# 3DAnimals/3DAnimals

Measured on AMD Instinct MI355X. Metric: train images/sec fwd+bwd @256x256 b16, higher is better.
Workload: dtype f32

## Files before the change

### 3danimals_amd/_lib.py

```python
from __future__ import annotations

import ctypes
import os

import torch

_HERE = os.path.dirname(os.path.abspath(__file__))
LIB_PATH = os.environ.get("A3D_LIB") or os.path.join(_HERE, "lib", "liba3d_hip.so")

_c_int, _c_float, _c_size_t, _p = ctypes.c_int, ctypes.c_float, ctypes.c_size_t, ctypes.c_void_p

SIGNATURES = {
    "a3d_version": (_c_int, []),
    "a3d_last_error": (ctypes.c_char_p, []),
    "a3d_bw_probe_fill": (_c_int, [_p, ctypes.c_int64, _p]),
    "a3d_bw_probe_read": (_c_int, [_p, ctypes.c_int64, _p, _p]),
    "a3d_dmtet_scratch_bytes": (_c_size_t, [_c_int, _c_int]),
    "a3d_dmtet_count": (_c_int, [_p, _p, _p, _c_int, _c_int, _p, _p, _p, _c_int, _c_int, _p, _p, _c_int, _p, _c_int, _p]),
    "a3d_dmtet_count_ordered": (_c_int, [_p, _c_int, _c_int, _c_int, _p, _p, _p, _p, _c_int, _p, _c_int, _p]),
    "a3d_dmtet_word_group_slots": (_c_int, []),
    "a3d_dmtet_word_group_bits": (_c_int, []),
    "a3d_dmtet_block_items": (_c_int, []),
    "a3d_dmtet_vertex_scratch_bytes": (_c_size_t, [_c_int]),
    "a3d_dmtet_gather_rows": (_c_int, [_p, _p, ctypes.c_int64, ctypes.c_int64, _c_int, _p, _p]),
# ... 125 lines not shown


class EstimateBonesArgs(ctypes.Structure):

    _fields_ = [("size", ctypes.c_uint32), ("N", ctypes.c_int32), ("pos", _p), ("bones", _p), ("nearest", _p), ("ok", _p), ("V", ctypes.c_int32),
                ("n_body", ctypes.c_int32), ("n_leg", ctypes.c_int32), ("body_mode_y_plus", ctypes.c_int32), ("use_y_threshold", ctypes.c_int32),
                ("y_threshold", ctypes.c_float), ("attach", ctypes.c_int32 * 4), ("blend", ctypes.c_float * 17), ("ramp", ctypes.c_float * 9), ("workspace", _p)]


class GbAux(ctypes.Structure):

    _fields_ = [("size", ctypes.c_uint32), ("reserved", ctypes.c_int32), ("tex_out", _p), ("img_out", _p), ("rows", ctypes.c_int64),
                ("pad_to", ctypes.c_int64)]


class DmtetEmitOpts(ctypes.Structure):

    _fields_ = [("size", ctypes.c_uint32), ("Nv", ctypes.c_int32), ("vertex_scratch", _p), ("surf_idx", _p), ("g_sdf_to_clear", _p), ("tri32", _p),
                ("topo_count", _p), ("topo_adj", _p), ("device_counts", _p), ("n_surf", ctypes.c_int32), ("topo_stride", ctypes.c_int32),
                ("use_block_lists", ctypes.c_int32), ("n_edge_blocks_listed", ctypes.c_int32), ("n_tet_blocks_listed", ctypes.c_int32),
                ("surf_bucket", ctypes.c_int32), ("surf_pts", _p)]


class TexDesc(ctypes.Structure):

    _fields_ = [("size", ctypes.c_uint32), ("C", ctypes.c_int32), ("tex_batch", ctypes.c_int32), ("filter", ctypes.c_int32), ("boundary", ctypes.c_int32),
                ("levels", ctypes.c_int32), ("height", ctypes.c_int32 * 16), ("width", ctypes.c_int32 * 16), ("level", _p * 16), ("grad", _p * 16)]


class EnvDesc(ctypes.Structure):

    _fields_ = [("size", ctypes.c_uint32), ("N", ctypes.c_int32), ("roughness", ctypes.c_float), ("costheta_cutoff", ctypes.c_float), ("src", _p),
                ("dst", _p), ("bounds", _p), ("area", _p)]


class BsdfDesc(ctypes.Structure):

    _fields_ = [("size", ctypes.c_uint32), ("op", ctypes.c_int32), ("variant", ctypes.c_int32), ("min_roughness", ctypes.c_float),
                ("ndim", ctypes.c_int32), ("reserved", ctypes.c_int32), ("shape", ctypes.c_int64 * 4), ("seg", ctypes.c_int64), ("in", _p * 6),
                ("stride", ctypes.c_int64 * 24), ("cstride", ctypes.c_int64 * 6), ("out", _p), ("scratch", _p), ("g_out", _p),
                ("g_mode", ctypes.c_int32 * 6), ("seg_div", ctypes.c_int64 * 6), ("g_in", _p * 6), ("g_final", _p * 6)]


BSDF_SIGNATURES = {
    "a3d_bsdf_rows": (ctypes.c_int64, [_p]),
    "a3d_bsdf_fwd": (_c_int, [_p, _p]),
    "a3d_bsdf_bwd": (_c_int, [_p, _p]),
    "a3d_image_loss_fwd": (_c_int, [_p, _p]),
    "a3d_image_loss_bwd": (_c_int, [_p, _p]),
}
BSDF_TILE = 1024
BSDF_MAX_DIMS = 4

ABI_VERSION = 404
_lib = None


class A3DError(RuntimeError):
    pass


def lib():
    global _lib
    if _lib is None:
        if not os.path.exists(LIB_PATH):
            raise A3DError(
                f"{LIB_PATH} is missing: build it with `python 3danimals_amd/csrc/build.py` "
                "(or __graft_entry__.build()).  There is no CPU fallback for the HIP hot path."
            )
        handle = ctypes.CDLL(LIB_PATH)
        for name, (res, args) in list(SIGNATURES.items()) + list(BSDF_SIGNATURES.items()):
            fn = getattr(handle, name)
            fn.restype, fn.argtypes = res, args
        if handle.a3d_version() != ABI_VERSION:
            raise A3DError(f"{LIB_PATH} has ABI version {handle.a3d_version()}, this package binds version {ABI_VERSION}: rebuild it "
                           "with `python 3danimals_amd/csrc/build.py`")
        _lib = handle
    return _lib


class KernelTimer:

    active = None

    def __init__(self):
        self.records = {}

    def __enter__(self):
        KernelTimer.active = self
        return self

    def __exit__(self, *exc):
        KernelTimer.active = None
        return False

    def summary(self):
        torch.cuda.synchronize()
        out = {}
        for name, pairs in self.records.items():
            ms = [a.elapsed_time(b) for a, b in pairs]
            out[name] = (len(ms), sum(ms) / max(len(ms), 1))
        return out


GUARD = int(os.environ.get("A3D_GUARD", "0") or 0)
GUARD_BYTES = 256
_GUARD_BYTE = 0xA5
_guard_live = []
guard_stats = dict(checks=0, buffers_checked=0, allocations=0)


def set_guard(level):
    global GUARD
    import importlib

    prev, GUARD = GUARD, int(level)
    ops = importlib.import_module(__package__ + ".ops")
    ops.torch = GuardedTorch(torch) if GUARD else torch
    if not GUARD:
        _guard_live.clear()
    return prev


def guarded_empty(shape, dtype, device, zero=False, site=""):
# ... 238 lines not shown
```

### 3danimals_amd/csrc/build.py

```python
import os
import subprocess
import sys
from concurrent.futures import ThreadPoolExecutor

HERE = os.path.dirname(os.path.abspath(__file__))
PKG = os.path.dirname(HERE)
LIB_DIR = os.path.join(PKG, "lib")
LIB = os.path.join(LIB_DIR, "liba3d_hip.so")
OBJ_DIR = os.path.join(HERE, "build")

SOURCES = {
    "common.hip": [],
    "dmtet.hip": ["-ffp-contract=off"],
    "skin.hip": [],
    "bones.hip": [],
    "normals.hip": ["-ffp-contract=off"],
    "raster.hip": ["-ffp-contract=off"],
    "cover.hip": [],
    "shade.hip": ["-ffp-contract=off"],
    "interp.hip": [],
    "gbuffer.hip": [],
    "segsum.hip": [],
    "losses.hip": [],
    "embed.hip": ["-ffp-contract=off"],
    "gemm.hip": [],
    "antialias.hip": ["-ffp-contract=off"],
    "topology.hip": [],
    "xfm.hip": ["-ffp-contract=off"],
    "texture.hip": ["-ffp-contract=off"],
    "envlight.hip": ["-ffp-contract=off"],
    "bsdf.hip": ["-ffp-contract=off"],
}
COMMON = ["--offload-arch=gfx950", "-O3", "-std=c++17", "-fPIC", "-fhip-fp32-correctly-rounded-divide-sqrt", "-Wall",
          "-Wno-unused-function"]


def _hipcc():
    for c in (os.environ.get("HIPCC"), "/opt/rocm/bin/hipcc", "hipcc"):
        if c and (os.path.isabs(c) and os.path.exists(c) or not os.path.isabs(c)):
            return c
    raise RuntimeError("hipcc not found")


def _stale(target, deps):
    if not os.path.exists(target):
        return True
    t = os.path.getmtime(target)
    return any(os.path.getmtime(d) > t for d in deps)


def build(force=False, verbose=True, profile=False, exp=False):
    assert not (profile and exp)
    lib = os.path.join(LIB_DIR, "liba3d_hip_prof.so") if profile else (os.path.join(LIB_DIR, "liba3d_hip_exp.so") if exp else LIB)
    obj_dir = os.path.join(OBJ_DIR, "prof") if profile else (os.path.join(OBJ_DIR, "exp") if exp else OBJ_DIR)
    os.makedirs(LIB_DIR, exist_ok=True)
    os.makedirs(obj_dir, exist_ok=True)
    hipcc = _hipcc()
    headers = sorted(os.path.join(HERE, f) for f in os.listdir(HERE) if f.endswith(".h")) + [os.path.join(os.path.dirname(PKG), "include", h) for h in ("a3d.h", "a3d_bsdf.h")] + [os.path.abspath(__file__)]
    jobs = []
    objs = []
    for src, extra in SOURCES.items():
        s = os.path.join(HERE, src)
        o = os.path.join(obj_dir, src.replace(".hip", ".o"))
        objs.append(o)
        if force or _stale(o, [s] + headers):
            jobs.append([hipcc, "-x", "hip", "-c", s, "-o", o] + COMMON + extra + (["-DA3D_PROFILE"] if profile else []) + (["-DA3D_EXPERIMENT"] if exp else []))

    def run(cmd):
        if verbose:
            print(" ".join(cmd), flush=True)
        subprocess.check_call(cmd)

    with ThreadPoolExecutor(max_workers=min(8, max(1, len(jobs)))) as ex:
        list(ex.map(run, jobs))
    if force or jobs or _stale(lib, objs):
        run([hipcc, "--offload-arch=gfx950", "-shared", "-fPIC", "-o", lib] + objs)
    return lib


if __name__ == "__main__":
    print(build(force="--force" in sys.argv, profile="--profile" in sys.argv, exp="--exp" in sys.argv))
```

### 3danimals_amd/hostnets.py

```python
from __future__ import annotations

import torch
import torch.nn as nn
import torch.nn.functional as F


REFERENCE_FORMULATION = False


def reference_formulation(enable=True):
    global REFERENCE_FORMULATION
    REFERENCE_FORMULATION = bool(enable)
    return REFERENCE_FORMULATION


def _activation(name):
    table = {"tanh": nn.Tanh, "sigmoid": nn.Sigmoid, "relu": nn.ReLU}
    if name not in table:
        raise NotImplementedError(name)
    return table[name]()


class HarmonicEmbedding(nn.Module):

# ... 2 lines not shown
        self.frequencies = scalar * (2.0 ** torch.arange(n_harmonic_functions))
        self._on_device = {}

    def _frequencies(self, device):
        f = self._on_device.get(device)
        if f is None:
            f = self._on_device[device] = self.frequencies.to(device)
        return f

    def forward(self, x):
        freq = self.frequencies.to(x.device) if REFERENCE_FORMULATION else self._frequencies(x.device)
        ang = (x[..., None] * freq).reshape(*x.shape[:-1], -1)
        return torch.cat((ang.sin(), ang.cos()), dim=-1)


USE_FIELD_STACK = True
SPLITK_MIN_ROWS = 65536
SPLITK_PARTS = 16


class _LinearSplitK(torch.autograd.Function):

    @staticmethod
    def forward(ctx, x, weight):
        ctx.save_for_backward(x, weight)
        return x.mm(weight.t())

    @staticmethod
    def backward(ctx, g):
        x, weight = ctx.saved_tensors
        gx = g.mm(weight) if ctx.needs_input_grad[0] else None
        gw = None
        if ctx.needs_input_grad[1]:
            gw = _split_k_weight_grad(g.contiguous(), x)
        return gx, gw


def _split_k_weight_grad(g, x):
    s, m = SPLITK_PARTS, x.shape[0]
    return torch.bmm(g.view(s, m // s, g.shape[1]).transpose(1, 2), x.view(s, m // s, x.shape[1])).sum(0)


_ZERO_BIAS = {}


def _zero_bias(x, weight):
    key = (x.device, weight.shape[0])
    b = _ZERO_BIAS.get(key)
    if b is None:
        b = _ZERO_BIAS[key] = torch.zeros(weight.shape[0], dtype=x.dtype, device=x.device)
    return b


class _LinearReLUSplitK(torch.autograd.Function):

    @staticmethod
    def forward(ctx, x, weight, bias):
        y = torch._addmm_activation(_zero_bias(x, weight) if bias is None else bias, x, weight.t(), use_gelu=False)
        ctx.save_for_backward(x, weight, y)
        return y

    @staticmethod
    def backward(ctx, g):
        x, weight, y = ctx.saved_tensors
        g = torch.ops.aten.threshold_backward(g.contiguous(), y, 0)
        gx = g.mm(weight) if ctx.needs_input_grad[0] else None
        gw = _split_k_weight_grad(g, x) if ctx.needs_input_grad[1] else None
        gb = g.sum(0) if ctx.needs_input_grad[2] else None
        return gx, gw, gb


class _FieldStack(torch.autograd.Function):

    @staticmethod
    def forward(ctx, x_emb, w_in, per_image, index, w_first, *hidden):
        from . import ops

        zero = _zero_bias(x_emb, w_in)
        ys = [torch._addmm_activation(zero, x_emb, w_in.t(), use_gelu=False)]
        if w_first is not None:
            y = ys[0].mm(w_first.t())
            ops.rows_add_relu_raw_(y, per_image, index)
            ys.append(y)
        for w in hidden:
            ys.append(torch._addmm_activation(zero, ys[-1], w.t(), use_gelu=False))
        ctx.save_for_backward(x_emb, w_in, index, w_first, *hidden, *ys)
        ctx.n_hidden, ctx.n_images = len(hidden), (per_image.shape[0] if per_image is not None else 0)
        return ys[-1]

    @staticmethod
    @torch.autograd.function.once_differentiable
    def backward(ctx, g):
        from . import ops

        saved = ctx.saved_tensors
        x_emb, w_in, index, w_first = saved[:4]
        hidden, ys = saved[4:4 + ctx.n_hidden], saved[4 + ctx.n_hidden:]
        g = torch.ops.aten.threshold_backward(g.contiguous(), ys[-1], 0)
        g_hidden = []
        for i in range(ctx.n_hidden - 1, -1, -1):
            y_prev = ys[len(ys) - ctx.n_hidden - 1 + i]
            g_hidden.append(_split_k_weight_grad(g, y_prev))
            g = ops.gemm_nn_relumask(g, hidden[i], y_prev)
        g_hidden.reverse()
        g_rows = g_first = None
        if w_first is not None:
            g_rows = ops.rows_segsum_raw(g, index, ctx.n_images)
            g_first = _split_k_weight_grad(g, ys[0])
            g = ops.gemm_nn_relumask(g, w_first, ys[0])
        g_in = _split_k_weight_grad(g, x_emb)
        g_x = g.mm(w_in) if ctx.needs_input_grad[0] else None
        return (g_x, g_in, g_rows, None, g_first, *g_hidden)


def _long_list(x, weight):
    return (x.is_cuda and x.dim() == 2 and x.shape[0] >= SPLITK_MIN_ROWS and x.shape[0] % SPLITK_PARTS == 0 and x.is_contiguous()
            and x.dtype == torch.float32 and torch.is_grad_enabled() and weight.requires_grad)


def linear(x, weight, bias=None):
    if bias is None and _long_list(x, weight):
        return _LinearSplitK.apply(x, weight)
    return F.linear(x, weight, bias)


def linear_relu(x, weight, bias=None):
    if _long_list(x, weight):
        return _LinearReLUSplitK.apply(x, weight, bias)
    if (x.is_cuda and x.dim() == 2 and x.shape[0] >= SPLITK_MIN_ROWS and x.dtype == torch.float32
            and not (torch.is_grad_enabled() and (x.requires_grad or weight.requires_grad or (bias is not None and bias.requires_grad)))):
        return torch._addmm_activation(_zero_bias(x, weight) if bias is None else bias, x, weight.t(), use_gelu=False)
    return torch.relu_(F.linear(x, weight, bias))


class MLP(nn.Module):

    def __init__(self, cin, cout, num_layers, nf=256, dropout=0, activation=None):
        super().__init__()
        assert num_layers >= 1
        dims = [cin] + [nf] * (num_layers - 1) + [cout]
        layers = []
        for i in range(num_layers):
            if i > 0:
                layers.append(nn.ReLU(inplace=True))
            layers.append(nn.Linear(dims[i], dims[i + 1], bias=False))
            if dropout and 0 < i < num_layers - 1:
                layers.append(nn.Dropout(dropout))
        if activation is not None:
            layers.append(_activation(activation))
        self.network = nn.Sequential(*layers)

    def forward(self, x, first_weight=None, per_image=None, index=None):
        if REFERENCE_FORMULATION and first_weight is None:
            return self.network(x)
        layers = list(self.network)
        i = 0
        if first_weight is not None:
            assert isinstance(layers[0], nn.Linear) and layers[0].bias is None
            x = linear(x, first_weight)
            if len(layers) > 1 and isinstance(layers[1], nn.ReLU) and x.is_cuda:
                from . import ops

                x = ops.rows_add_relu_(x, per_image, index)
                i = 2
            else:
                x = x + per_image[index]
                i = 1
        while i < len(layers):
            layer = layers[i]
            if isinstance(layer, nn.Linear) and i + 1 < len(layers) and isinstance(layers[i + 1], nn.ReLU):
                x = linear_relu(x, layer.weight, layer.bias)
                i += 2
                continue
            x = linear(x, layer.weight, layer.bias) if isinstance(layer, nn.Linear) else layer(x)
            i += 1
        return x


class CoordMLP(nn.Module):

    def __init__(self, cin, cout, num_layers, nf=256, dropout=0, activation=None, min_max=None, n_harmonic_functions=10,
                 embedder_scalar=1, embed_concat_pts=True, extra_feat_dim=0, symmetrize=False, in_layer_relu=False):
        super().__init__()
        self.extra_feat_dim = extra_feat_dim
        if n_harmonic_functions > 0:
            self.embedder = HarmonicEmbedding(n_harmonic_functions, embedder_scalar)
            dim_in = cin * 2 * n_harmonic_functions + (cin if embed_concat_pts else 0)
            self.embed_concat_pts = embed_concat_pts
        else:
            self.embedder = None
            dim_in = cin
        self.in_layer = nn.Linear(dim_in, nf)
        self.relu = nn.ReLU(inplace=True)
        self.mlp = MLP(nf + extra_feat_dim, cout, num_layers, nf, dropout, activation)
        self.symmetrize = symmetrize
        if min_max is not None:
            self.register_buffer("min_max", min_max)
        else:
            self.min_max = None
        self.bsdf = None
        self.in_layer_relu = in_layer_relu

    @property
    def indexed_feat(self):
        return not REFERENCE_FORMULATION

    def forward(self, x, feat=None, feat_index=None):
        assert (feat is None and self.extra_feat_dim == 0) or (feat.shape[-1] == self.extra_feat_dim)
        if REFERENCE_FORMULATION:
            return self._forward_reference(x, feat if feat_index is None or feat is None else feat[feat_index])
        if feat_index is not None and feat is not None and x.dim() == 2 and isinstance(self.mlp.network[0], nn.Linear) \
                and self.mlp.network[0].bias is None:
            return self._forward_indexed(x, feat, feat_index)
        if feat_index is not None and feat is not None:
            feat = feat[feat_index]
        if feat is None and self._stack_ok(x, False):
            return self._stacked(x, None, None)
        if feat is None and self._fused_input_ok(x):
            out = self.mlp(self._fused_input(x))
# ... 27 lines not shown
            x = torch.stack([xs.abs(), ys, zs], -1)
        x_in = x
        if self.embedder is not None:
            x_in = self.embedder(x)
            if self.embed_concat_pts:
                x_in = torch.cat([x, x_in], -1)
        x_in = self.in_layer(x_in)
        if self.in_layer_relu:
            x_in = self.relu(x_in)
        if feat is not None:
            for _ in range(x_in.dim() - feat.dim()):
                feat = feat.unsqueeze(1)
            x_in = torch.cat([x_in, feat.expand(*x_in.shape[:-1], -1)], dim=-1)
        out = self.mlp(self.relu(x_in))
        if self.min_max is not None:
            out = out * (self.min_max[:, 1] - self.min_max[:, 0]) + self.min_max[:, 0]
        return out

    def _fused_input_ok(self, x):
        return (x.is_cuda and x.dim() == 2 and x.shape[1] == 3 and x.shape[0] >= SPLITK_MIN_ROWS and x.dtype == torch.float32
                and self.embedder is not None and self.embed_concat_pts and self.in_layer.bias is not None)

    def _fused_input(self, x):
        from . import ops

        h = ops.harmonic_embed(x, self.embedder._frequencies(x.device), symmetrize=self.symmetrize, ones=True)
        weight = torch.cat([self.in_layer.weight, self.in_layer.bias[:, None]], dim=1)
        return linear_relu(h, weight, None)

    def _stack_ok(self, x, with_feat):
        if not (USE_FIELD_STACK and self._fused_input_ok(x) and torch.is_grad_enabled() and x.shape[0] % SPLITK_PARTS == 0
                and self.in_layer.weight.requires_grad and self.in_layer.weight.shape[0] == 256):
            return False
        layers = list(self.mlp.network)
        n_pairs = 0
        while 2 * n_pairs + 1 < len(layers) and isinstance(layers[2 * n_pairs], nn.Linear) and isinstance(layers[2 * n_pairs + 1], nn.ReLU):
            lin = layers[2 * n_pairs]
            want_in = 256 + (self.extra_feat_dim if (with_feat and n_pairs == 0) else 0)
            if lin.bias is not None or tuple(lin.weight.shape) != (256, want_in):
                return False
            n_pairs += 1
        return n_pairs >= 1

    def _stacked(self, x, feat, feat_index):
        from . import ops

        layers = list(self.mlp.network)
        pairs, i = [], 0
        while i + 1 < len(layers) and isinstance(layers[i], nn.Linear) and isinstance(layers[i + 1], nn.ReLU):
            pairs.append(layers[i])
            i += 2
        x_emb = ops.harmonic_embed(x, self.embedder._frequencies(x.device), symmetrize=self.symmetrize, ones=True)
        w_in = torch.cat([self.in_layer.weight, self.in_layer.bias[:, None]], dim=1)
        if feat is not None:
            first = pairs[0].weight
            per_image = F.linear(torch.relu(feat), first[:, 256:])
            h = _FieldStack.apply(x_emb, w_in, per_image, feat_index, first[:, :256].contiguous(), *[l.weight for l in pairs[1:]])
        else:
            h = _FieldStack.apply(x_emb, w_in, None, None, None, *[l.weight for l in pairs])
        for layer in layers[i:]:
            h = linear(h, layer.weight, layer.bias) if isinstance(layer, nn.Linear) else layer(h)
        if self.min_max is not None:
            h = h * (self.min_max[:, 1] - self.min_max[:, 0]) + self.min_max[:, 0]
        return h

    def _forward_indexed(self, x, feat, feat_index):
        if self._stack_ok(x, True):
            return self._stacked(x, feat, feat_index)
        if self._fused_input_ok(x):
            h = self._fused_input(x)
        else:
            if self.symmetrize:
                x = torch.cat([x[..., :1].abs(), x[..., 1:]], -1)
            h = x
            if self.embedder is not None:
                h = self.embedder(x)
                if self.embed_concat_pts:
                    h = torch.cat([x, h], -1)
            h = linear_relu(h, self.in_layer.weight, self.in_layer.bias)
        nf = h.shape[-1]
        weight = self.mlp.network[0].weight
        per_image = F.linear(torch.relu(feat), weight[:, nf:])
        out = self.mlp(h, first_weight=weight[:, :nf].contiguous(), per_image=per_image, index=feat_index)
        if self.min_max is not None:
            out = out * (self.min_max[:, 1] - self.min_max[:, 0]) + self.min_max[:, 0]
        return out

    def sample(self, x, feat=None, feat_index=None):
        return self.forward(x, feat, feat_index)


class Linear_Mod(nn.Module):
    def __init__(self, in_features, out_features, bias=True):
        super().__init__()
        self.in_features, self.out_features = in_features, out_features
        self.weight = nn.Parameter(torch.empty((out_features, in_features)))
        if bias:
            self.bias = nn.Parameter(torch.empty(out_features))
        else:
            self.register_parameter("bias", None)
        nn.init.kaiming_uniform_(self.weight, a=5 ** 0.5)
        if self.bias is not None:
            fan_in, _ = nn.init._calculate_fan_in_and_fan_out(self.weight)
            bound = 1 / fan_in ** 0.5 if fan_in > 0 else 0
            nn.init.uniform_(self.bias, -bound, bound)

    def forward(self, x, style):
        if style.dim() > 1:
            style = style.reshape(-1, style.shape[-1])[0]
        weight = self.weight * style.unsqueeze(0)
        weight = weight / ((weight * weight).sum(dim=-1, keepdim=True) + 1e-5).sqrt()
        return F.linear(x, weight, self.bias)

# ... 64 lines not shown
```

### 3danimals_amd/ops.py

```python
from __future__ import annotations

import ctypes
import math
import os
from collections import OrderedDict

import torch

from . import _lib
from ._lib import call, f32c, f32h, ptr, require_device, stream


class _IdentityCache:

    def __init__(self, maxsize=8):
        self.maxsize = maxsize
        self.data = OrderedDict()

    @staticmethod
    def key(t):
        return (t.data_ptr(), tuple(t.shape), t.dtype, t._version)

    def get(self, t, make):
        k = self.key(t)
# ... 1221 lines not shown
    def forward(ctx, t, img):
        ctx.save_for_backward(img)
        ctx.b = t.shape[0]
        return t.index_select(0, img)

    @staticmethod
    def backward(ctx, g):
        (img,) = ctx.saved_tensors
        g = f32c(g)
        P, C = g.shape[0], int(math.prod(g.shape[1:]))
        out = torch.empty((ctx.b,) + tuple(g.shape[1:]), dtype=torch.float32, device=g.device)
        call("a3d_rows_segsum", ptr(g), ptr(img), P, C, ctx.b, ptr(out), stream(), tag=f"[C{C}]")
        return out, None


CHECK_SORTED_INDEX = False


def _assert_sorted(img):
    if CHECK_SORTED_INDEX and img is not None and img.numel() > 1:
        torch._assert_async((img[1:] >= img[:-1]).all(), "point -> image index must be non-decreasing")


def rows_per_point(t, img):
    require_device(t, img, what="rows_per_point")
    _assert_sorted(img)
    return _RowsPerPoint.apply(t, img) if (t.requires_grad and torch.is_grad_enabled()) else t.index_select(0, img)


class _RowsAddReLU(torch.autograd.Function):

    @staticmethod
    def forward(ctx, y, rows, img):
        require_device(y, rows, img, what="rows_add_relu")
        assert y.is_contiguous() and y.dtype == torch.float32 and y.dim() == 2 and rows.shape[1] == y.shape[1] and img.shape[0] == y.shape[0]
        rows = f32c(rows)
        call("a3d_rows_add_relu_fwd", ptr(y), ptr(rows), ptr(img), y.shape[0], y.shape[1], rows.shape[0], stream(), tag=f"[C{y.shape[1]}]")
        ctx.mark_dirty(y)
        ctx.save_for_backward(y, img)
        ctx.b = rows.shape[0]
        return y

    @staticmethod
    def backward(ctx, g):
        y, img = ctx.saved_tensors
        g = f32c(g)
        g_pre = torch.empty_like(g)
        g_rows = torch.empty((ctx.b, y.shape[1]), dtype=torch.float32, device=g.device)
        call("a3d_rows_add_relu_bwd", ptr(g), ptr(y), ptr(img), y.shape[0], y.shape[1], ctx.b, ptr(g_pre), ptr(g_rows), stream(),
             tag=f"[C{y.shape[1]}]")
        return g_pre, g_rows, None


def rows_add_relu_raw_(y, rows, img):
    call("a3d_rows_add_relu_fwd", ptr(y), ptr(f32h(rows)), ptr(img), y.shape[0], y.shape[1], rows.shape[0], stream(), tag=f"[C{y.shape[1]}]")
    return y


def rows_segsum_raw(g, img, b):
    _assert_sorted(img)
    g = f32c(g)
    out = torch.empty((b, g.shape[1]), dtype=torch.float32, device=g.device)
    call("a3d_rows_segsum", ptr(g), ptr(img), g.shape[0], g.shape[1], b, ptr(out), stream(), tag=f"[C{g.shape[1]}]")
    return out


def rows_add_relu_(y, rows, img):
    _assert_sorted(img)
    return _RowsAddReLU.apply(y, rows, img)


class AAAnalysis:

    def __init__(self, rast, clip, topo: AATopology, defer=False):
        require_device(rast, clip, what="antialias")
        ensure_resolved(rast)
        self.rast, self.clip, self.topo = f32c(rast.detach()), f32c(clip.detach()), topo
        B, H, W = rast.shape[:3]
        self.B, self.H, self.W = B, H, W
        shards = _lib.lib().a3d_aa_shards()
        self.capacity = _lib.lib().a3d_aa_capacity(B, H, W)
        dev = rast.device
        self.work = torch.empty((self.capacity, 4), dtype=torch.int32, device=dev)
        prep = _aa_prepared.take(self.rast)
        self.prepared = prep is not None and prep[0] == _IdentityCache.key(self.clip)
        if self.prepared:
            self.screen, self.count = prep[1], prep[2]
        else:
            self.count = torch.empty((shards,), dtype=torch.int32, device=dev)
            self.screen = torch.empty((self.clip.shape[0], self.clip.shape[1], 2), dtype=torch.float32, device=dev)
        self.pending = True
        if not (defer and self.prepared and topo.tri.shape[0] > 0):
            self.ensure()

    def ride_args(self):
        if self.pending and self.B > 65535:
            self.ensure()
        if not self.pending:
            return None
        topo, lists = self.topo, getattr(self.topo, "lists", None)
        return _lib.AaRide(size=ctypes.sizeof(_lib.AaRide), clip_batch=self.clip.shape[0], rast=ptr(self.rast), screen=ptr(self.screen),
                           tri=ptr(topo.tri), opp=ptr(topo.opp), off=ptr(None if lists is None else lists.off),
                           adj=ptr(None if lists is None else lists.adj), V=self.clip.shape[1], F=topo.tri.shape[0],
                           lists_stride=0 if lists is None else lists.stride)

    def ensure(self):
# ... 295 lines not shown
        ctx.save_for_backward(flow, flow_gt, both, scale)
        ctx.dims = (B, F, H, W)
        return loss

    @staticmethod
    def backward(ctx, g_loss):
        flow, flow_gt, both, scale = ctx.saved_tensors
        B, F, H, W = ctx.dims
        g_flow = torch.empty((B * F, H, W, 2), dtype=torch.float32, device=flow.device)
        call("a3d_flow_loss_bwd", ptr(f32h(g_loss)), ptr(scale), ptr(flow), flow.stride(2), ptr(flow_gt), ptr(both), B, F, H, W, ptr(g_flow), stream())
        return g_flow, None, None, None, None


def flow_loss(flow_nchw, flow_gt, both, batch, num_frames):
    return _FlowLoss.apply(flow_nchw.permute(0, 2, 3, 1), flow_gt, both, int(batch), int(num_frames))


class _HarmonicEmbed(torch.autograd.Function):
    @staticmethod
    def forward(ctx, x, freq, symmetrize, ones):
        require_device(x, freq, what="harmonic_embed")
        x, freq = f32c(x), f32c(freq)
        P, n = x.shape[0], freq.shape[0]
        assert x.shape == (P, 3)
        out = torch.empty((P, 3 + 6 * n + int(ones)), dtype=torch.float32, device=x.device)
        call("a3d_harmonic_embed_fwd", ptr(x), ptr(freq), n, int(symmetrize), int(ones), P, ptr(out), stream())
        ctx.save_for_backward(x, freq)
        ctx.cfg = (int(symmetrize), int(ones))
        return out

    @staticmethod
    @torch.autograd.function.once_differentiable
    def backward(ctx, g):
        x, freq = ctx.saved_tensors
        g_x = torch.empty_like(x)
        call("a3d_harmonic_embed_bwd", ptr(f32h(g)), ptr(x), ptr(freq), freq.shape[0], ctx.cfg[0], ctx.cfg[1], x.shape[0], ptr(g_x), stream())
        return g_x, None, None, None


def harmonic_embed(x, freq, symmetrize=False, ones=False):
    return _HarmonicEmbed.apply(x, freq, symmetrize, ones)


def gemm_nn_relumask(a, b, x=None):
    require_device(a, b, what="gemm_nn_relumask")
    a, b = f32c(a), f32c(b)
    M, K = a.shape
    assert b.shape == (K, 256) and K % 32 == 0 and (x is None or (x.shape == (M, 256) and x.is_contiguous() and x.dtype == torch.float32))
    c = torch.empty((M, 256), dtype=torch.float32, device=a.device)
    call("a3d_gemm_nn_relumask", ptr(a), ptr(b), ptr(x), M, 256, K, ptr(c), stream())
    return c


_TEX_FILTERS = {"nearest": 0, "linear": 1, "linear-mipmap-nearest": 2, "linear-mipmap-linear": 3}
_TEX_BOUNDARIES = {"wrap": 0, "clamp": 1, "zero": 2, "cube": 3}
TEX_MAX_LEVELS = 16


def texture_filter_mode(filter_mode, uv_da=None, mip_level_bias=None):
    if filter_mode == "auto":
        return "linear-mipmap-linear" if (uv_da is not None or mip_level_bias is not None) else "linear"
    if filter_mode not in _TEX_FILTERS:
        raise ValueError(f"texture: unknown filter_mode {filter_mode!r}")
    return filter_mode


def texture_mip_sizes(height, width, max_mip_level=None):
    sizes = [(int(height), int(width))]
    top = TEX_MAX_LEVELS - 1 if max_mip_level is None else min(int(max_mip_level), TEX_MAX_LEVELS - 1)
    while len(sizes) - 1 < top:
        h, w = sizes[-1]
        if (h == 1 and w == 1) or (h > 1 and h % 2) or (w > 1 and w % 2):
            break
        sizes.append((max(h // 2, 1), max(w // 2, 1)))
    return sizes


def _tex_hw(t, cube):
    if cube:
        if t.dim() != 5 or t.shape[1] != 6 or t.shape[2] != t.shape[3]:
            raise ValueError(f"texture: a cube level must have shape [Bt, 6, S, S, C], got {list(t.shape)}")
        return t.shape[0], t.shape[2], t.shape[3], t.shape[4]
    if t.dim() != 4:
        raise ValueError(f"texture: a 2-D level must have shape [Bt, H, W, C], got {list(t.shape)}")
    return t.shape[0], t.shape[1], t.shape[2], t.shape[3]


def _tex_desc(levels, C, tex_batch, filt, boundary, grads=None):
    d = _lib.TexDesc(size=ctypes.sizeof(_lib.TexDesc), C=C, tex_batch=tex_batch, filter=filt, boundary=boundary, levels=len(levels))
    cube = boundary == _TEX_BOUNDARIES["cube"]
    for l, t in enumerate(levels):
        d.height[l], d.width[l] = (t.shape[2], t.shape[3]) if cube else (t.shape[1], t.shape[2])
        d.level[l] = t.data_ptr()
        if grads is not None and grads[l] is not None:
            d.grad[l] = grads[l].data_ptr()
    return d


class _TextureMip(torch.autograd.Function):

    @staticmethod
    def forward(ctx, tex, sizes, cube):
        require_device(tex, what="texture_construct_mip")
        tex = f32c(tex)
        Bt, _, _, C = _tex_hw(tex, cube)
        lead = (Bt, 6) if cube else (Bt,)
# ... 477 lines not shown
```

Baseline: 1026.

## Add fused MFMA kernels for field MLP linear+ReLU and output head

Adds a new HIP source with an MFMA-based 256x256 linear+ReLU kernel that can also fuse the per-image row add, plus fused head forward and backward kernels. The head kernels fold the small output projection, sigmoid and min-max scaling into one pass, and the backward also computes the ReLU-masked input gradient and weight-gradient partials, followed by a reduce. The field stack is rewired to use these paths when the shapes match. The aim is to remove separate GEMM, elementwise and rows-add launches and the memory traffic between them. The cost is extra custom code and slightly different fp32 summation order.

```diff
diff --git a/3danimals_amd/_lib.py b/3danimals_amd/_lib.py
--- a/3danimals_amd/_lib.py
+++ b/3danimals_amd/_lib.py
@@ -201,6 +201,16 @@
 BSDF_TILE = 1024
 BSDF_MAX_DIMS = 4
 
+FIELD_SIGNATURES = {
+    "a3d_field_linear_relu_fwd": (_c_int, [_p, _p, _p, _p, ctypes.c_int64, _c_int, _c_int, _c_int, _p, _p]),
+    "a3d_field_head_fwd": (_c_int, [_p, _p, _p, ctypes.c_int64, _c_int, _c_int, _c_int, _c_int, _p, _p, _p]),
+    "a3d_field_head_bwd": (_c_int, [_p, _p, _p, _p, _p, ctypes.c_int64, _c_int, _c_int, _c_int, _c_int, _p, _p, _p, _p]),
+}
+FIELD_WIDTH = 256
+FIELD_HEAD_MAX = 16
+FIELD_GROUPS_MAX = 1024
+FIELD_ACTS = {None: 0, "sigmoid": 1}
+
 ABI_VERSION = 404
 _lib = None
 
@@ -218,7 +228,7 @@
                 "(or __graft_entry__.build()).  There is no CPU fallback for the HIP hot path."
             )
         handle = ctypes.CDLL(LIB_PATH)
-        for name, (res, args) in list(SIGNATURES.items()) + list(BSDF_SIGNATURES.items()):
+        for name, (res, args) in list(SIGNATURES.items()) + list(BSDF_SIGNATURES.items()) + list(FIELD_SIGNATURES.items()):
             fn = getattr(handle, name)
             fn.restype, fn.argtypes = res, args
         if handle.a3d_version() != ABI_VERSION:
diff --git a/3danimals_amd/csrc/build.py b/3danimals_amd/csrc/build.py
--- a/3danimals_amd/csrc/build.py
+++ b/3danimals_amd/csrc/build.py
@@ -30,6 +30,7 @@
     "texture.hip": ["-ffp-contract=off"],
     "envlight.hip": ["-ffp-contract=off"],
     "bsdf.hip": ["-ffp-contract=off"],
+    "fields.hip": [],
 }
 COMMON = ["--offload-arch=gfx950", "-O3", "-std=c++17", "-fPIC", "-fhip-fp32-correctly-rounded-divide-sqrt", "-Wall",
           "-Wno-unused-function"]
@@ -56,7 +57,7 @@
     os.makedirs(LIB_DIR, exist_ok=True)
     os.makedirs(obj_dir, exist_ok=True)
     hipcc = _hipcc()
-    headers = sorted(os.path.join(HERE, f) for f in os.listdir(HERE) if f.endswith(".h")) + [os.path.join(os.path.dirname(PKG), "include", h) for h in ("a3d.h", "a3d_bsdf.h")] + [os.path.abspath(__file__)]
+    headers = sorted(os.path.join(HERE, f) for f in os.listdir(HERE) if f.endswith(".h")) + [os.path.join(os.path.dirname(PKG), "include", h) for h in ("a3d.h", "a3d_bsdf.h", "a3d_fields.h")] + [os.path.abspath(__file__)]
     jobs = []
     objs = []
     for src, extra in SOURCES.items():
diff --git a/3danimals_amd/csrc/fields.hip b/3danimals_amd/csrc/fields.hip
--- /dev/null
+++ b/3danimals_amd/csrc/fields.hip
@@ -0,0 +1,351 @@
+#include "a3d_common.h"
+#include "../../include/a3d_fields.h"
+
+namespace {
+
+typedef float f32x16 __attribute__((ext_vector_type(16)));
+typedef float f32x4 __attribute__((ext_vector_type(4)));
+
+constexpr int FD_W = A3D_FIELD_WIDTH;
+
+constexpr int FL_BN = 128, FL_WAVES = 16, FL_LDS_BYTES = FD_W * FL_BN * 4;
+
+template <bool ROWS>
+__global__ __launch_bounds__(64 * FL_WAVES, 1) void fd_linear_relu_kernel(const float* __restrict__ x, const float* __restrict__ W,
+                                                                          const float* __restrict__ rows, const long long* __restrict__ index,
+                                                                          int M, int B, float* __restrict__ y) {
+    constexpr int K = FD_W, TN = 4;
+    extern __shared__ float Bs[];
+    const int tid = threadIdx.x, lane = tid & 63, wave = tid >> 6;
+    const int half = blockIdx.x & 1, bid = blockIdx.x >> 1, nb = gridDim.x >> 1;
+    const int n0 = half * FL_BN;
+#pragma unroll
+    for (int i = 0; i < 8; ++i) {
+        const int f = tid + 1024 * i;
+        const int n = (f & 31) + 32 * ((f >> 6) & 3), q = ((f >> 5) & 1) + 2 * (f >> 8);
+        const f32x4 w = *reinterpret_cast<const f32x4*>(W + (long long)(n0 + n) * K + 4 * q);
+        float* d = Bs + (4 * q) * FL_BN + n;
+        d[0] = w.x; d[FL_BN] = w.y; d[2 * FL_BN] = w.z; d[3 * FL_BN] = w.w;
+    }
+    __syncthreads();
+
+    const int row = lane & 31, kh = lane >> 5;
+    const int n_tiles = (M + 31) >> 5;
+    const int stride = nb * FL_WAVES;
+    const float* b_lane = Bs + 4 * kh * FL_BN + row;
+    for (int t = (wave >> 2) * (nb * 4) + bid * 4 + (wave & 3); t < n_tiles; t += stride) {
+        const long long m0 = 32ll * t;
+        const long long mr = m0 + row < M ? m0 + row : M - 1;
+        const float* a_lane = x + mr * K + 4 * kh;
+        f32x16 acc[TN];
+#pragma unroll
+        for (int j = 0; j < TN; ++j)
+#pragma unroll
+            for (int r = 0; r < 16; ++r) acc[j][r] = 0.f;
+
+        f32x4 an[4];
+#pragma unroll
+        for (int i = 0; i < 4; ++i) an[i] = *reinterpret_cast<const f32x4*>(a_lane + 8 * i);
+#pragma unroll 1
+        for (int c = 0; c < 8; ++c) {
+            f32x4 av[4];
+#pragma unroll
+            for (int i = 0; i < 4; ++i) av[i] = an[i];
+            {
+                const int cn = c + 1 < 8 ? c + 1 : 0;
+#pragma unroll
+                for (int i = 0; i < 4; ++i) an[i] = *reinterpret_cast<const f32x4*>(a_lane + 32 * cn + 8 * i);
+            }
+            const float* bc = b_lane + (32 * c) * FL_BN;
+#pragma unroll
+            for (int g = 0; g < 4; ++g)
+#pragma unroll
+                for (int u = 0; u < 4; ++u) {
+                    const float* bp = bc + (8 * g + u) * FL_BN;
+#pragma unroll
+                    for (int j = 0; j < TN; ++j) acc[j] = __builtin_amdgcn_mfma_f32_32x32x2f32(av[g][u], bp[32 * j], acc[j], 0, 0, 0);
+                }
+        }
+        const long long mrow = m0 + 4 * kh;
+#pragma unroll
+        for (int r = 0; r < 16; ++r) {
+            const long long m = mrow + (r & 3) + 8 * (r >> 2);
+            if (m < M) {
+                const float* add = nullptr;
+                if (ROWS) {
+                    const long long b = index[m];
+                    if ((unsigned long long)b < (unsigned long long)B) add = rows + b * FD_W + n0 + row;
+                }
+#pragma unroll
+                for (int j = 0; j < TN; ++j) {
+                    float v = acc[j][r];
+                    if (ROWS && add) v += add[32 * j];
+                    y[m * FD_W + n0 + 32 * j + row] = fmaxf(v, 0.f);
+                }
+            }
+        }
+    }
+}
+
+constexpr int FH_WAVES = 8, FH_ROWS = 16, FH_LD = FD_W + 4, FH_TILE = FH_ROWS * FH_LD;
+constexpr int FH_FWD_LDS_BYTES = FH_WAVES * FH_TILE * 4;
+constexpr int FH_BWD_LDS_BYTES = (FH_WAVES + 1) * FH_TILE * 4;
+
+__device__ __forceinline__ void fh_load_tile(const float* __restrict__ y, long long m0, int M, int lane, f32x4 (&v)[FH_ROWS]) {
+#pragma unroll
+    for (int r = 0; r < FH_ROWS; ++r) {
+        const long long m = m0 + r < M ? m0 + r : M - 1;
+        v[r] = __builtin_nontemporal_load(reinterpret_cast<const f32x4*>(y + m * FD_W) + lane);
+    }
+}
+
+template <bool SIGMOID>
+__global__ __launch_bounds__(64 * FH_WAVES, 1) void fd_head_fwd_kernel(const float* __restrict__ y, const float* __restrict__ Wh,
+                                                                       const float* __restrict__ min_max, int M, int C,
+                                                                       float* __restrict__ out, float* __restrict__ act_val) {
+    extern __shared__ float lds[];
+    const int tid = threadIdx.x, lane = tid & 63, wave = tid >> 6, n = lane & 15, j = lane >> 4;
+    float* tile = lds + wave * FH_TILE;
+    f32x4 wreg[16];
+    const f32x4 zero4 = {0.f, 0.f, 0.f, 0.f};
+#pragma unroll
+    for (int t = 0; t < 16; ++t) wreg[t] = n < C ? *reinterpret_cast<const f32x4*>(Wh + n * FD_W + 16 * t + 4 * j) : zero4;
+    float lo = 0.f, scale = 1.f;
+    if (min_max && n < C) lo = min_max[2 * n], scale = min_max[2 * n + 1] - lo;
+
+    const int n_tiles = (M + FH_ROWS - 1) / FH_ROWS, stride = gridDim.x * FH_WAVES;
+    int t0 = blockIdx.x * FH_WAVES + wave;
+    f32x4 v[FH_ROWS];
+    if (t0 < n_tiles) fh_load_tile(y, (long long)FH_ROWS * t0, M, lane, v);
+    for (; t0 < n_tiles; t0 += stride) {
+        const long long m0 = (long long)FH_ROWS * t0;
+#pragma unroll
+        for (int r = 0; r < FH_ROWS; ++r) *reinterpret_cast<f32x4*>(tile + r * FH_LD + 4 * lane) = v[r];
+        if (t0 + stride < n_tiles) fh_load_tile(y, (long long)FH_ROWS * (t0 + stride), M, lane, v);
+        f32x4 acc = zero4;
+#pragma unroll
+        for (int t = 0; t < 16; ++t) {
+            const f32x4 a = *reinterpret_cast<const f32x4*>(tile + n * FH_LD + 16 * t + 4 * j);
+#pragma unroll
+            for (int s = 0; s < 4; ++s) acc = __builtin_amdgcn_mfma_f32_16x16x4f32(a[s], wreg[t][s], acc, 0, 0, 0);
+        }
+        if (n < C) {
+#pragma unroll
+            for (int r = 0; r < 4; ++r) {
+                const long long m = m0 + 4 * j + r;
+                if (m < M) {
+                    float a = acc[r];
+                    if (SIGMOID) a = 1.f / (1.f + expf(-a));
+                    if (act_val) act_val[m * C + n] = a;
+                    out[m * C + n] = min_max ? __fadd_rn(__fmul_rn(a, scale), lo) : a;
+                }
+            }
+        }
+    }
+}
+
+template <bool SIGMOID>
+__global__ __launch_bounds__(64 * FH_WAVES, 1) void fd_head_bwd_kernel(const float* __restrict__ g_out, const float* __restrict__ act_val,
+                                                                       const float* __restrict__ y, const float* __restrict__ Wh,
+                                                                       const float* __restrict__ min_max, int M, int C,
+                                                                       float* __restrict__ g_y, float* __restrict__ partials) {
+    extern __shared__ float lds[];
+    const int tid = threadIdx.x, lane = tid & 63, wave = tid >> 6, n = lane & 15, j = lane >> 4;
+    float* Wl = lds;
+    float* tile = lds + (1 + wave) * FH_TILE;
+#pragma unroll
+    for (int i = 0; i < 16 * FD_W / (64 * FH_WAVES); ++i) {
+        const int f = tid + 64 * FH_WAVES * i, c = f >> 8, k = f & 255;
+        Wl[c * FH_LD + k] = c < C ? Wh[f] : 0.f;
+    }
+    __syncthreads();
+
+    float sc_a[4], sc_d = 0.f;
+#pragma unroll
+    for (int s = 0; s < 4; ++s) sc_a[s] = 4 * j + s < C ? (min_max ? min_max[2 * (4 * j + s) + 1] - min_max[2 * (4 * j + s)] : 1.f) : 0.f;
+    if (n < C) sc_d = min_max ? min_max[2 * n + 1] - min_max[2 * n] : 1.f;
+    auto g_pre = [&](long long m, int c, float sc) -> float {
+        if (m >= M || c >= C) return 0.f;
+        float g = g_out[m * C + c] * sc;
+        if (SIGMOID) {
+            const float a = act_val[m * C + c];
+            g *= (1.f - a) * a;
+        }
+        return g;
+    };
+
+    const f32x4 zero4 = {0.f, 0.f, 0.f, 0.f};
+    f32x4 dw[16];
+#pragma unroll
+    for (int t = 0; t < 16; ++t) dw[t] = zero4;
+
+    const int n_tiles = (M + FH_ROWS - 1) / FH_ROWS, stride = gridDim.x * FH_WAVES;
+    int t0 = blockIdx.x * FH_WAVES + wave;
+    f32x4 v[FH_ROWS];
+    if (t0 < n_tiles) fh_load_tile(y, (long long)FH_ROWS * t0, M, lane, v);
+    for (; t0 < n_tiles; t0 += stride) {
+        const long long m0 = (long long)FH_ROWS * t0;
+#pragma unroll
+        for (int r = 0; r < FH_ROWS; ++r) *reinterpret_cast<f32x4*>(tile + r * FH_LD + 4 * lane) = v[r];
+        if (t0 + stride < n_tiles) fh_load_tile(y, (long long)FH_ROWS * (t0 + stride), M, lane, v);
+        float ga[4], gd[4];
+#pragma unroll
+        for (int s = 0; s < 4; ++s) {
+            ga[s] = g_pre(m0 + n, 4 * j + s, sc_a[s]);
+            gd[s] = g_pre(m0 + 4 * j + s, n, sc_d);
+        }
+#pragma unroll
+        for (int t = 0; t < 16; ++t) {
+            float* yp = tile + (4 * j) * FH_LD + 16 * t + n;
+            const float* wp = Wl + (4 * j) * FH_LD + 16 * t + n;
+            float ys[4];
+#pragma unroll
+            for (int s = 0; s < 4; ++s) ys[s] = yp[s * FH_LD];
+            f32x4 acc = zero4;
+#pragma unroll
+            for (int s = 0; s < 4; ++s) acc = __builtin_amdgcn_mfma_f32_16x16x4f32(ga[s], wp[s * FH_LD], acc, 0, 0, 0);
+#pragma unroll
+            for (int s = 0; s < 4; ++s) dw[t] = __builtin_amdgcn_mfma_f32_16x16x4f32(gd[s], ys[s], dw[t], 0, 0, 0);
+#pragma unroll
+            for (int s = 0; s < 4; ++s) yp[s * FH_LD] = ys[s] > 0.f ? acc[s] : 0.f;
+        }
+#pragma unroll
+        for (int r = 0; r < FH_ROWS; ++r)
+            if (m0 + r < M)
+                reinterpret_cast<f32x4*>(g_y + (m0 + r) * FD_W)[lane] = *reinterpret_cast<const f32x4*>(tile + r * FH_LD + 4 * lane);
+    }
+#pragma unroll
+    for (int t = 0; t < 16; ++t)
+#pragma unroll
+        for (int r = 0; r < 4; ++r) tile[(4 * j + r) * FH_LD + 16 * t + n] = dw[t][r];
+    __syncthreads();
+#pragma unroll
+    for (int i = 0; i < 16 * FD_W / (64 * FH_WAVES); ++i) {
+        const int f = tid + 64 * FH_WAVES * i, c = f >> 8, k = f & 255;
+        if (c < C) {
+            float s = 0.f;
+#pragma unroll
+            for (int w = 0; w < FH_WAVES; ++w) s += lds[(1 + w) * FH_TILE + c * FH_LD + k];
+            partials[((long long)blockIdx.x * C + c) * FD_W + k] = s;
+        }
+    }
+}
+
+__global__ __launch_bounds__(256) void fd_head_reduce_kernel(const float* __restrict__ partials, int G, int n_out, float* __restrict__ dW) {
+    __shared__ float red[16][17];
+    const int tx = threadIdx.x & 15, sub = threadIdx.x >> 4;
+    const int o = blockIdx.x * 16 + tx;
+    float s = 0.f;
+    if (o < n_out) {
+        int g = sub;
+        for (; g + 16 * 7 < G; g += 16 * 8) {
+            float p[8];
+#pragma unroll
+            for (int i = 0; i < 8; ++i) p[i] = partials[(long long)(g + 16 * i) * n_out + o];
+#pragma unroll
+            for (int i = 0; i < 8; ++i) s += p[i];
+        }
+        for (; g < G; g += 16) s += partials[(long long)g * n_out + o];
+    }
+    red[sub][tx] = s;
+    __syncthreads();
+    if (sub == 0 && o < n_out) {
+        float a = 0.f;
+#pragma unroll
+        for (int i = 0; i < 16; ++i) a += red[i][tx];
+        dW[o] = a;
+    }
+}
+
+template <typename Kern>
+int fd_allow_lds(Kern kernel, int bytes) {
+    A3D_HIP(hipFuncSetAttribute(reinterpret_cast<const void*>(kernel), hipFuncAttributeMaxDynamicSharedMemorySize, bytes));
+    return A3D_OK;
+}
+
+}
+
+extern "C" int a3d_field_linear_relu_fwd(const float* x, const float* W, const float* rows, const int64_t* index, int64_t M, int N, int K, int B,
+                                         float* y, a3d_stream_t stream) {
+    A3D_CHECK_ARG(M >= 0 && M < 0x7fffffffll && N == FD_W && K == FD_W);
+    A3D_CHECK_ARG((rows == nullptr) == (index == nullptr) && (rows == nullptr || B > 0));
+    if (M == 0) return A3D_OK;
+    A3D_CHECK_ARG(x && W && y);
+    static int n_cu_of[64] = {0};
+    int dev = 0;
+    A3D_HIP(hipGetDevice(&dev));
+    A3D_CHECK_ARG(dev >= 0 && dev < 64);
+    if (!n_cu_of[dev]) {
+        int n = 0;
+        A3D_HIP(hipDeviceGetAttribute(&n, hipDeviceAttributeMultiprocessorCount, dev));
+        if (int rc = fd_allow_lds(fd_linear_relu_kernel<true>, FL_LDS_BYTES)) return rc;
+        if (int rc = fd_allow_lds(fd_linear_relu_kernel<false>, FL_LDS_BYTES)) return rc;
+        n_cu_of[dev] = n;
+    }
+    A3D_CHECK_ARG(n_cu_of[dev] >= 2);
+    const dim3 grid(n_cu_of[dev] & ~1), block(64 * FL_WAVES);
+    hipStream_t s = (hipStream_t)stream;
+    if (rows) hipLaunchKernelGGL(fd_linear_relu_kernel<true>, grid, block, FL_LDS_BYTES, s, x, W, rows, (const long long*)index, (int)M, B, y);
+    else hipLaunchKernelGGL(fd_linear_relu_kernel<false>, grid, block, FL_LDS_BYTES, s, x, W, rows, (const long long*)index, (int)M, B, y);
+    A3D_LAUNCH_CHECK();
+    return A3D_OK;
+}
+
+static int fd_head_check(const char* func, int64_t M, int K, int C, int act, int groups) {
+    if (!(M >= 0 && M < 0x7fffffffll && K == FD_W && C >= 1 && C <= A3D_FIELD_HEAD_MAX && groups >= 1 && groups <= A3D_FIELD_GROUPS_MAX &&
+          (act == A3D_FIELD_ACT_NONE || act == A3D_FIELD_ACT_SIGMOID))) {
+        a3d_set_error("%s: invalid argument: 0 <= M < 2^31, K == 256, 1 <= C <= 16, 1 <= groups <= 1024, act in {0, 1} (M %lld K %d C %d act %d groups %d)",
+                      func, (long long)M, K, C, act, groups);
+        return A3D_EINVAL;
+    }
+    return A3D_OK;
+}
+
+extern "C" int a3d_field_head_fwd(const float* y, const float* W_h, const float* min_max, int64_t M, int K, int C, int act, int groups, float* out,
+                                  float* act_val, a3d_stream_t stream) {
+    if (int rc = fd_head_check(__func__, M, K, C, act, groups)) return rc;
+    if (M == 0) return A3D_OK;
+    A3D_CHECK_ARG(y && W_h && out);
+    static bool allowed[64] = {false};
+    int dev = 0;
+    A3D_HIP(hipGetDevice(&dev));
+    A3D_CHECK_ARG(dev >= 0 && dev < 64);
+    if (!allowed[dev]) {
+        if (int rc = fd_allow_lds(fd_head_fwd_kernel<true>, FH_FWD_LDS_BYTES)) return rc;
+        if (int rc = fd_allow_lds(fd_head_fwd_kernel<false>, FH_FWD_LDS_BYTES)) return rc;
+        allowed[dev] = true;
+    }
+    const dim3 grid(groups), block(64 * FH_WAVES);
+    hipStream_t s = (hipStream_t)stream;
+    if (act == A3D_FIELD_ACT_SIGMOID) hipLaunchKernelGGL(fd_head_fwd_kernel<true>, grid, block, FH_FWD_LDS_BYTES, s, y, W_h, min_max, (int)M, C, out, act_val);
+    else hipLaunchKernelGGL(fd_head_fwd_kernel<false>, grid, block, FH_FWD_LDS_BYTES, s, y, W_h, min_max, (int)M, C, out, act_val);
+    A3D_LAUNCH_CHECK();
+    return A3D_OK;
+}
+
+extern "C" int a3d_field_head_bwd(const float* g_out, const float* act_val, const float* y, const float* W_h, const float* min_max, int64_t M,
+                                  int K, int C, int act, int groups, float* g_y, float* partials, float* g_W_h, a3d_stream_t stream) {
+    if (int rc = fd_head_check(__func__, M, K, C, act, groups)) return rc;
+    if (M == 0) return A3D_OK;
+    hipStream_t s = (hipStream_t)stream;
+    A3D_CHECK_ARG(g_out && y && W_h && g_y && partials && g_W_h);
+    A3D_CHECK_ARG(act == A3D_FIELD_ACT_NONE || act_val != nullptr);
+    static bool allowed[64] = {false};
+    int dev = 0;
+    A3D_HIP(hipGetDevice(&dev));
+    A3D_CHECK_ARG(dev >= 0 && dev < 64);
+    if (!allowed[dev]) {
+        if (int rc = fd_allow_lds(fd_head_bwd_kernel<true>, FH_BWD_LDS_BYTES)) return rc;
+        if (int rc = fd_allow_lds(fd_head_bwd_kernel<false>, FH_BWD_LDS_BYTES)) return rc;
+        allowed[dev] = true;
+    }
+    const dim3 grid(groups), block(64 * FH_WAVES);
+    if (act == A3D_FIELD_ACT_SIGMOID)
+        hipLaunchKernelGGL(fd_head_bwd_kernel<true>, grid, block, FH_BWD_LDS_BYTES, s, g_out, act_val, y, W_h, min_max, (int)M, C, g_y, partials);
+    else
+        hipLaunchKernelGGL(fd_head_bwd_kernel<false>, grid, block, FH_BWD_LDS_BYTES, s, g_out, act_val, y, W_h, min_max, (int)M, C, g_y, partials);
+    A3D_LAUNCH_CHECK();
+    hipLaunchKernelGGL(fd_head_reduce_kernel, dim3(a3d_div_up(C * FD_W, 16)), dim3(256), 0, s, partials, groups, C * FD_W, g_W_h);
+    A3D_LAUNCH_CHECK();
+    return A3D_OK;
+}
diff --git a/3danimals_amd/hostnets.py b/3danimals_amd/hostnets.py
--- a/3danimals_amd/hostnets.py
+++ b/3danimals_amd/hostnets.py
@@ -78,11 +78,24 @@
     return b
 
 
+def _own_forward_gemm(x, weight, bias=None):
+    return (bias is None and x.is_cuda and x.dim() == 2 and tuple(weight.shape) == (256, 256) and x.shape[1] == 256 and x.is_contiguous()
+            and weight.is_contiguous() and x.dtype == torch.float32 and weight.dtype == torch.float32)
+
+
+def _linear_relu_forward(x, weight, bias=None):
+    if _own_forward_gemm(x, weight, bias):
+        from . import ops
+
+        return ops.field_linear_relu(x.detach(), weight.detach())
+    return torch._addmm_activation(_zero_bias(x, weight) if bias is None else bias, x, weight.t(), use_gelu=False)
+
+
 class _LinearReLUSplitK(torch.autograd.Function):
 
     @staticmethod
     def forward(ctx, x, weight, bias):
-        y = torch._addmm_activation(_zero_bias(x, weight) if bias is None else bias, x, weight.t(), use_gelu=False)
+        y = _linear_relu_forward(x, weight, bias)
         ctx.save_for_backward(x, weight, y)
         return y
 
@@ -96,23 +109,50 @@
         return gx, gw, gb
 
 
+class _LinearRowsReLU(torch.autograd.Function):
+
+    @staticmethod
+    def forward(ctx, x, weight, rows, index):
+        from . import ops
+
+        y = ops.field_linear_relu(x, weight, rows, index)
+        ctx.save_for_backward(x, weight, index, y)
+        ctx.n_images = rows.shape[0]
+        return y
+
+    @staticmethod
+    @torch.autograd.function.once_differentiable
+    def backward(ctx, g):
+        from . import ops
+
+        x, weight, index, y = ctx.saved_tensors
+        g, g_rows = ops.rows_add_relu_bwd_raw(g, y, index, ctx.n_images)
+        gx = g.mm(weight) if ctx.needs_input_grad[0] else None
+        gw = _split_k_weight_grad(g, x) if ctx.needs_input_grad[1] else None
+        return gx, gw, g_rows, None
+
+
 class _FieldStack(torch.autograd.Function):
 
     @staticmethod
-    def forward(ctx, x_emb, w_in, per_image, index, w_first, *hidden):
+    def forward(ctx, x_emb, w_in, per_image, index, w_first, w_head, activation, min_max, *hidden):
         from . import ops
 
         zero = _zero_bias(x_emb, w_in)
         ys = [torch._addmm_activation(zero, x_emb, w_in.t(), use_gelu=False)]
         if w_first is not None:
-            y = ys[0].mm(w_first.t())
-            ops.rows_add_relu_raw_(y, per_image, index)
-            ys.append(y)
+            ys.append(ops.field_linear_relu(ys[0], w_first, per_image, index))
         for w in hidden:
-            ys.append(torch._addmm_activation(zero, ys[-1], w.t(), use_gelu=False))
-        ctx.save_for_backward(x_emb, w_in, index, w_first, *hidden, *ys)
+            ys.append(ops.field_linear_relu(ys[-1], w.contiguous()))
         ctx.n_hidden, ctx.n_images = len(hidden), (per_image.shape[0] if per_image is not None else 0)
-        return ys[-1]
+        ctx.head = None
+        if w_head is None:
+            ctx.save_for_backward(x_emb, w_in, index, w_first, *hidden, *ys)
+            return ys[-1]
+        out, act_val = ops.field_head_fwd(ys[-1], w_head, min_max, activation)
+        ctx.head = (activation, min_max, act_val is not None)
+        ctx.save_for_backward(x_emb, w_in, index, w_first, *hidden, *ys, w_head, *([act_val] if act_val is not None else []))
+        return out
 
     @staticmethod
     @torch.autograd.function.once_differentiable
@@ -122,7 +162,13 @@
         saved = ctx.saved_tensors
         x_emb, w_in, index, w_first = saved[:4]
         hidden, ys = saved[4:4 + ctx.n_hidden], saved[4 + ctx.n_hidden:]
-        g = torch.ops.aten.threshold_backward(g.contiguous(), ys[-1], 0)
+        g_head = None
+        if ctx.head is None:
+            g = torch.ops.aten.threshold_backward(g.contiguous(), ys[-1], 0)
+        else:
+            activation, min_max, has_act = ctx.head
+            ys, w_head, act_val = (ys[:-2], ys[-2], ys[-1]) if has_act else (ys[:-1], ys[-1], None)
+            g, g_head = ops.field_head_bwd(g, act_val, ys[-1], w_head, min_max, activation)
         g_hidden = []
         for i in range(ctx.n_hidden - 1, -1, -1):
             y_prev = ys[len(ys) - ctx.n_hidden - 1 + i]
@@ -136,7 +182,7 @@
             g = ops.gemm_nn_relumask(g, w_first, ys[0])
         g_in = _split_k_weight_grad(g, x_emb)
         g_x = g.mm(w_in) if ctx.needs_input_grad[0] else None
-        return (g_x, g_in, g_rows, None, g_first, *g_hidden)
+        return (g_x, g_in, g_rows, None, g_first, g_head, None, None, *g_hidden)
 
 
 def _long_list(x, weight):
@@ -155,7 +201,7 @@
         return _LinearReLUSplitK.apply(x, weight, bias)
     if (x.is_cuda and x.dim() == 2 and x.shape[0] >= SPLITK_MIN_ROWS and x.dtype == torch.float32
             and not (torch.is_grad_enabled() and (x.requires_grad or weight.requires_grad or (bias is not None and bias.requires_grad)))):
-        return torch._addmm_activation(_zero_bias(x, weight) if bias is None else bias, x, weight.t(), use_gelu=False)
+        return _linear_relu_forward(x, weight, bias)
     return torch.relu_(F.linear(x, weight, bias))
 
 
@@ -183,14 +229,18 @@
         i = 0
         if first_weight is not None:
             assert isinstance(layers[0], nn.Linear) and layers[0].bias is None
-            x = linear(x, first_weight)
-            if len(layers) > 1 and isinstance(layers[1], nn.ReLU) and x.is_cuda:
+            relu_next = len(layers) > 1 and isinstance(layers[1], nn.ReLU)
+            if (relu_next and _long_list(x, first_weight) and _own_forward_gemm(x, first_weight) and index.dtype == torch.int64
+                    and index.is_contiguous() and tuple(per_image.shape[1:]) == (256,)):
+                x = _LinearRowsReLU.apply(x, first_weight, per_image, index)
+                i = 2
+            elif relu_next and x.is_cuda:
                 from . import ops
 
-                x = ops.rows_add_relu_(x, per_image, index)
+                x = ops.rows_add_relu_(linear(x, first_weight), per_image, index)
                 i = 2
             else:
-                x = x + per_image[index]
+                x = linear(x, first_weight) + per_image[index]
                 i = 1
         while i < len(layers):
             layer = layers[i]
@@ -324,13 +374,19 @@
             i += 2
         x_emb = ops.harmonic_embed(x, self.embedder._frequencies(x.device), symmetrize=self.symmetrize, ones=True)
         w_in = torch.cat([self.in_layer.weight, self.in_layer.bias[:, None]], dim=1)
+        tail, head = layers[i:], (None, None, None)
+        if (tail and isinstance(tail[0], nn.Linear) and tail[0].bias is None and tail[0].weight.shape[0] <= 16 and tail[0].weight.shape[1] == 256
+                and (len(tail) == 1 or (len(tail) == 2 and isinstance(tail[1], nn.Sigmoid)))):
+            head = (tail[0].weight, "sigmoid" if len(tail) == 2 else None, self.min_max)
         if feat is not None:
             first = pairs[0].weight
             per_image = F.linear(torch.relu(feat), first[:, 256:])
-            h = _FieldStack.apply(x_emb, w_in, per_image, feat_index, first[:, :256].contiguous(), *[l.weight for l in pairs[1:]])
-        else:
-            h = _FieldStack.apply(x_emb, w_in, None, None, None, *[l.weight for l in pairs])
-        for layer in layers[i:]:
+            h = _FieldStack.apply(x_emb, w_in, per_image, feat_index, first[:, :256].contiguous(), *head, *[l.weight for l in pairs[1:]])
+        else:
+            h = _FieldStack.apply(x_emb, w_in, None, None, None, *head, *[l.weight for l in pairs])
+        if head[0] is not None:
+            return h
+        for layer in tail:
             h = linear(h, layer.weight, layer.bias) if isinstance(layer, nn.Linear) else layer(h)
         if self.min_max is not None:
             h = h * (self.min_max[:, 1] - self.min_max[:, 0]) + self.min_max[:, 0]
diff --git a/3danimals_amd/ops.py b/3danimals_amd/ops.py
--- a/3danimals_amd/ops.py
+++ b/3danimals_amd/ops.py
@@ -1297,6 +1297,15 @@
         return g_pre, g_rows, None
 
 
+def rows_add_relu_bwd_raw(g, y, img, b):
+    _assert_sorted(img)
+    g = f32c(g)
+    g_pre = torch.empty_like(g)
+    g_rows = torch.empty((b, y.shape[1]), dtype=torch.float32, device=g.device)
+    call("a3d_rows_add_relu_bwd", ptr(g), ptr(y), ptr(img), y.shape[0], y.shape[1], b, ptr(g_pre), ptr(g_rows), stream(), tag=f"[C{y.shape[1]}]")
+    return g_pre, g_rows
+
+
 def rows_add_relu_raw_(y, rows, img):
     call("a3d_rows_add_relu_fwd", ptr(y), ptr(f32h(rows)), ptr(img), y.shape[0], y.shape[1], rows.shape[0], stream(), tag=f"[C{y.shape[1]}]")
     return y
@@ -1698,6 +1707,62 @@
     return c
 
 
+def field_linear_relu(x, weight, rows=None, index=None):
+    require_device(x, weight, rows, index, what="field_linear_relu")
+    M = x.shape[0]
+    assert x.shape == (M, 256) and weight.shape == (256, 256) and x.dtype == weight.dtype == torch.float32 and x.is_contiguous() \
+        and weight.is_contiguous() and (rows is None) == (index is None)
+    assert rows is None or (rows.dim() == 2 and rows.shape[1] == 256 and index.shape == (M,) and index.dtype == torch.int64 and index.is_contiguous())
+    y = torch.empty((M, 256), dtype=torch.float32, device=x.device)
+    call("a3d_field_linear_relu_fwd", ptr(x), ptr(weight), ptr(None if rows is None else f32h(rows)), ptr(index), M, 256, 256,
+         0 if rows is None else rows.shape[0], ptr(y), stream(), tag="[rows]" if rows is not None else "")
+    return y
+
+
+_FIELD_GROUPS = {}
+
+
+def _field_groups(device):
+    g = _FIELD_GROUPS.get(device)
+    if g is None:
+        g = _FIELD_GROUPS[device] = max(1, min(_lib.FIELD_GROUPS_MAX, torch.cuda.get_device_properties(device).multi_processor_count))
+    return g
+
+
+def _field_head_args(y, w_head, min_max, activation):
+    M, C = y.shape[0], w_head.shape[0]
+    if activation not in _lib.FIELD_ACTS:
+        raise ValueError(f"field head: activation {activation!r} has no kernel")
+    assert y.shape == (M, 256) and y.dtype == torch.float32 and y.is_contiguous() and w_head.shape == (C, 256) and 1 <= C <= _lib.FIELD_HEAD_MAX
+    assert min_max is None or tuple(min_max.shape) == (C, 2)
+    return M, C, _lib.FIELD_ACTS[activation]
+
+
+def field_head_fwd(y, w_head, min_max=None, activation=None):
+    require_device(y, w_head, min_max, what="field_head_fwd")
+    M, C, act = _field_head_args(y, w_head, min_max, activation)
+    out = torch.empty((M, C), dtype=torch.float32, device=y.device)
+    act_val = torch.empty_like(out) if (act and min_max is not None) else None
+    call("a3d_field_head_fwd", ptr(y), ptr(f32h(w_head)), ptr(None if min_max is None else f32h(min_max)), M, 256, C, act, _field_groups(y.device),
+         ptr(out), ptr(act_val), stream(), tag=f"[C{C}]")
+    return out, ((out if act_val is None else act_val) if act else None)
+
+
+def field_head_bwd(g_out, act_val, y, w_head, min_max=None, activation=None):
+    require_device(g_out, y, w_head, min_max, act_val, what="field_head_bwd")
+    M, C, act = _field_head_args(y, w_head, min_max, activation)
+    assert g_out.shape == (M, C) and (not act or (act_val is not None and act_val.shape == (M, C) and act_val.is_contiguous()))
+    if M == 0:
+        return torch.empty((0, 256), dtype=torch.float32, device=y.device), torch.zeros((C, 256), dtype=torch.float32, device=y.device)
+    groups = _field_groups(y.device)
+    g_y = torch.empty((M, 256), dtype=torch.float32, device=y.device)
+    partials = torch.empty((groups, C, 256), dtype=torch.float32, device=y.device)
+    g_w = torch.empty((C, 256), dtype=torch.float32, device=y.device)
+    call("a3d_field_head_bwd", ptr(f32h(g_out)), ptr(act_val if act else None), ptr(y), ptr(f32h(w_head)), ptr(None if min_max is None else f32h(min_max)),
+         M, 256, C, act, groups, ptr(g_y), ptr(partials), ptr(g_w), stream(), tag=f"[C{C}]")
+    return g_y, g_w
+
+
 _TEX_FILTERS = {"nearest": 0, "linear": 1, "linear-mipmap-nearest": 2, "linear-mipmap-linear": 3}
 _TEX_BOUNDARIES = {"wrap": 0, "clamp": 1, "zero": 2, "cube": 3}
 TEX_MAX_LEVELS = 16
diff --git a/include/a3d_fields.h b/include/a3d_fields.h
--- /dev/null
+++ b/include/a3d_fields.h
@@ -0,0 +1,29 @@
+#ifndef A3D_FIELDS_H
+#define A3D_FIELDS_H
+
+#include "a3d.h"
+
+#ifdef __cplusplus
+extern "C" {
+#endif
+
+#define A3D_FIELD_WIDTH 256
+#define A3D_FIELD_HEAD_MAX 16
+#define A3D_FIELD_GROUPS_MAX 1024
+
+#define A3D_FIELD_ACT_NONE 0
+#define A3D_FIELD_ACT_SIGMOID 1
+
+int a3d_field_linear_relu_fwd(const float* x, const float* W, const float* rows, const int64_t* index, int64_t M, int N, int K, int B,
+                              float* y, a3d_stream_t stream);
+
+int a3d_field_head_fwd(const float* y, const float* W_h, const float* min_max, int64_t M, int K, int C, int act, int groups, float* out,
+                       float* act_val, a3d_stream_t stream);
+
+int a3d_field_head_bwd(const float* g_out, const float* act_val, const float* y, const float* W_h, const float* min_max, int64_t M, int K,
+                       int C, int act, int groups, float* g_y, float* partials, float* g_W_h, a3d_stream_t stream);
+
+#ifdef __cplusplus
+}
+#endif
+#endif
```

Measured after the change: 1022 (median of 2 runs). No clear change (-0.4%).
